# taha-kms/CLASSMATE-RAG

Hardware: AMD Instinct MI355X
Metric: hybrid queries/sec + recall@10 vs reference, 10M×768 chunks, 1/2/4/8 GPU (higher is better)
Workload: dtype fp32-accurate E5 (K10 f16x3 MFMA) + int8/f16/f64 dense + f64 BM25

## Files before the change

classmate-rag_amd/csrc/cm_bm25.hip:

```cpp
#include "cm_common.h"

#include <hipcub/hipcub.hpp>

#include <algorithm>
#include <cmath>
#include <cstdlib>
#include <numeric>
#include <vector>

namespace cm {

constexpr int kRange = 1024;
constexpr int kBmThreads = 256;
constexpr int kBoundsGroup = 8;
constexpr int kMergeThreads = 1024;
constexpr int kMergePer = 16;
constexpr int kTermLanesQd = 16;

__device__ inline int64_t lhead(int q, int64_t r, int64_t nr) { return (int64_t)q * nr + r; }
__host__ __device__ inline int64_t lheads_total(int nq, int64_t nr) { return (int64_t)nq * nr; }
__device__ inline int64_t lslot(int q, int64_t r, int64_t nr, int64_t nl, int k, int j) {
  return j == 0 ? lhead(q, r, nr) : nl + ((int64_t)q * nr + r) * (k - 1) + (j - 1);
}

// ... 937 lines not shown
  const int64_t d = df[i];
  double v = 0.0;
  if (t >= 0 && t < vocab && d > 0 && nc <= log_n) {
    v = logtab[nc - d] - logtab[d];
    if (v < 0) {
      const double e = eps_dev ? *eps_dev : __builtin_nan("");
      if (e != e) atomicOr(status, 1);
      v = e;
    }
  }
  q_idf[i] = v;
}

}

using namespace cm;

struct cm_bm25 {
  int dev = 0;
  hipStream_t stream = nullptr;
  int64_t ndocs = 0, npost = 0;
  int32_t vocab = 0;
  int64_t n_live = 0, sum_len = 0;
  double avgdl = 0.0, eps = 0.0;
  bool empty_vocab = false;
  DevBuf term_off, post_doc, post_tf, post_pos, dl, live, idf;
  DevBuf headtf, head_id;
  DevBuf logtab;
  int64_t log_n = -1;
  DevBuf head_maxtf, range_mindl;
  DevBuf blk_maxtf, blk_mindl;
  DevBuf blk_maxr;
  DevBuf blk16_maxr;
  double maxr_avgdl = 0.0;
  int32_t path = 0;
  int32_t last_rescored = 0;
  int32_t nhead = 0;
  int64_t npad = 0;
  int32_t lut_dmin = 0;
  double head_min_frac = 1.0 / 128.0;
  int64_t head_max_bytes = 8ll << 30;
  std::vector<double> idf_host;
  DevBuf ws, qbuf, obuf, allow_buf, tmp;
  KernelTimer timer;
  KernelTimer timer_b;
};

namespace {

inline double bm25_idf(int64_t n, int64_t df) {
  return std::log((double)(n - df) + 0.5) - std::log((double)df + 0.5);
}

int compute_idf_table(cm_bm25 *h, const std::vector<int32_t> &df, const std::vector<int32_t> &order) {
  h->idf_host.assign(h->vocab, 0.0);
  h->empty_vocab = false;
  h->eps = 0.0;
  h->avgdl = h->n_live ? (double)h->sum_len / (double)h->n_live : 0.0;
  if (h->n_live == 0) return CM_OK;
  if (order.empty()) {
    h->empty_vocab = true;
    return CM_OK;
  }
  double idf_sum = 0.0;
  for (int32_t t : order) {
    const double v = bm25_idf(h->n_live, df[t]);
// ... 52 lines not shown
    int32_t *dcand = h->tmp.as<int32_t>(), *dsat = dcand + cand.size();
    CM_HIP(hipMemcpyAsync(dcand, cand.data(), cand.size() * 4, hipMemcpyHostToDevice, h->stream));
    CM_HIP(hipMemsetAsync(dsat, 0, cand.size() * 4, h->stream));
    hipLaunchKernelGGL(bm25_head_sat_kernel, dim3(16, (unsigned)cand.size()), dim3(256), 0, h->stream, dcand,
                       (int)cand.size(), h->term_off.as<int64_t>(), h->post_tf.as<uint16_t>(), dsat);
    CM_HIP(hipGetLastError());
    std::vector<int32_t> sat(cand.size());
    CM_HIP(hipMemcpyAsync(sat.data(), dsat, cand.size() * 4, hipMemcpyDeviceToHost, h->stream));
    CM_HIP(hipStreamSynchronize(h->stream));
    size_t o = 0;
    for (size_t i = 0; i < cand.size(); ++i)
      if (!sat[i]) cand[o++] = cand[i];
    cand.resize(o);
  }
  const int64_t max_h = h->head_max_bytes / h->npad;
  if ((int64_t)cand.size() > max_h) cand.resize((size_t)std::max<int64_t>(max_h, 0));
  std::vector<int32_t> hid((size_t)std::max(h->vocab, 1), -1);
  for (size_t i = 0; i < cand.size(); ++i) hid[cand[i]] = (int32_t)i;
  if ((rc = h->head_id.ensure((size_t)std::max(h->vocab, 1) * 4))) return rc;
  CM_HIP(hipMemcpyAsync(h->head_id.ptr, hid.data(), (size_t)std::max(h->vocab, 1) * 4, hipMemcpyHostToDevice,
                        h->stream));
  if (!cand.empty()) {
    const size_t bytes = cand.size() * (size_t)h->npad;
    if ((rc = h->headtf.ensure(bytes)) || (rc = h->tmp.ensure(cand.size() * 4))) return rc;
    CM_HIP(hipMemsetAsync(h->headtf.ptr, 0, bytes, h->stream));
    CM_HIP(hipMemcpyAsync(h->tmp.ptr, cand.data(), cand.size() * 4, hipMemcpyHostToDevice, h->stream));
    hipLaunchKernelGGL(bm25_head_fill_kernel, dim3(64, (unsigned)cand.size()), dim3(256), 0, h->stream,
                       h->tmp.as<int32_t>(), (int)cand.size(), h->term_off.as<int64_t>(), h->post_doc.as<int32_t>(),
                       h->post_tf.as<uint16_t>(), h->headtf.as<uint8_t>(), h->npad);
    CM_HIP(hipGetLastError());
    CM_HIP(hipStreamSynchronize(h->stream));
  }
  h->nhead = (int32_t)cand.size();
  const int64_t nr = std::max<int64_t>(1, ceil_div(h->ndocs, kRange));
  if ((rc = h->range_mindl.ensure((size_t)nr * 4))) return rc;
  hipLaunchKernelGGL(bm25_range_mindl_kernel, dim3((unsigned)ceil_div(nr * 64, 256)), dim3(256), 0, h->stream,
                     h->dl.as<int32_t>(), h->ndocs, (int)nr, h->range_mindl.as<int32_t>());
  CM_HIP(hipGetLastError());
  const int64_t nblk = nr * (kRange / 64);
  if ((rc = h->blk_mindl.ensure((size_t)nblk * 4))) return rc;
  hipLaunchKernelGGL(bm25_blk_mindl_kernel, dim3((unsigned)ceil_div(nblk, 256)), dim3(256), 0, h->stream,
                     h->dl.as<int32_t>(), h->ndocs, nblk, h->blk_mindl.as<int32_t>());
  CM_HIP(hipGetLastError());
  if (h->nhead) {
    if ((rc = h->head_maxtf.ensure((size_t)h->nhead * nr)) || (rc = h->blk_maxtf.ensure((size_t)h->nhead * nblk)))
      return rc;
    hipLaunchKernelGGL(bm25_head_max_kernel, dim3((unsigned)ceil_div((int64_t)h->nhead * nr * 64, 256)), dim3(256), 0,
                       h->stream, h->headtf.as<uint8_t>(), h->npad, (int)nr, h->nhead, h->head_maxtf.as<uint8_t>());
    CM_HIP(hipGetLastError());
    hipLaunchKernelGGL(bm25_blk_max_kernel, dim3((unsigned)ceil_div((int64_t)h->nhead * nblk, 256)), dim3(256), 0,
                       h->stream, h->headtf.as<uint8_t>(), h->npad, nblk, h->nhead, h->blk_maxtf.as<uint8_t>());
    CM_HIP(hipGetLastError());
    h->maxr_avgdl = h->avgdl > 0.0 ? h->avgdl * 1.05 : 0.0;
    if (h->maxr_avgdl > 0.0) {
      if ((rc = h->blk_maxr.ensure((size_t)h->nhead * nblk)) || (rc = h->blk16_maxr.ensure((size_t)h->nhead * nblk * 4)))
        return rc;
      hipLaunchKernelGGL(bm25_blk_maxratio_kernel, dim3((unsigned)ceil_div((int64_t)h->nhead * nblk, 256)),
                         dim3(256), 0, h->stream, h->headtf.as<uint8_t>(), h->npad, h->dl.as<int32_t>(), h->ndocs,
                         nblk, h->nhead, h->maxr_avgdl, h->blk_maxr.as<uint8_t>(), 64);
      CM_HIP(hipGetLastError());
      hipLaunchKernelGGL(bm25_blk_maxratio_kernel, dim3((unsigned)ceil_div((int64_t)h->nhead * nblk * 4, 256)),
                         dim3(256), 0, h->stream, h->headtf.as<uint8_t>(), h->npad, h->dl.as<int32_t>(), h->ndocs,
                         nblk * 4, h->nhead, h->maxr_avgdl, h->blk16_maxr.as<uint8_t>(), 16);
      CM_HIP(hipGetLastError());
    }
  }
// ... 67 lines not shown
  off += 256;
  w.df = reinterpret_cast<int64_t *>(p + off);
  off += round_up((int64_t)std::max(total_terms, 1) * 8, 256);
  w.qd_code = reinterpret_cast<int32_t *>(p + off);
  off += round_up((int64_t)std::max(nq, 1) * kTermLanes * 4, 256);
  w.qd_idf = reinterpret_cast<double *>(p + off);
  off += round_up((int64_t)std::max(nq, 1) * kTermLanes * 8, 256);
  w.qd_tb = reinterpret_cast<int32_t *>(p + off);
  off += round_up((int64_t)std::max(nq, 1) * 4, 256);
  w.qd_len = reinterpret_cast<int32_t *>(p + off);
  off += round_up((int64_t)std::max(nq, 1) * 4, 256);
  w.qd_term = reinterpret_cast<int32_t *>(p + off);
  off += round_up((int64_t)std::max(nq, 1) * kTermLanes * 4, 256);
  w.total = off;
  return w;
}

#ifndef K2A_RPW
#define K2A_RPW 4
#endif
#ifndef K2B_GRID
#define K2B_GRID 2048
#endif
int bm25_launch_core(cm_bm25 *h, const int32_t *q_terms_dev, const int32_t *q_off_dev, int nq, int total_terms, int k,
                     const uint32_t *allow_dev, const BmWs &w, double *score_dev, int64_t *row_dev, hipStream_t st,
                     hipEvent_t gate = nullptr) {
  int rc;
  const double *avgdl = w.avgdl;
  const int nr = (int)std::max<int64_t>(1, ceil_div(h->ndocs, kRange));
  if (nr > kMergePer * kMergeThreads) CM_FAIL(CM_EUNSUPPORTED, "BM25 shard too large (> 16.7M docs)");
  const int ngroups = (nr + 1 + kBoundsGroup - 1) / kBoundsGroup;
  const int64_t nb = (int64_t)total_terms * ngroups;
  const bool prune = h->path != 1 && !(bm25_debug_flags() & 4);
  if (nq > 0) {
    hipLaunchKernelGGL(bm25_qcand_kernel, dim3((unsigned)ceil_div(nq, 256)), dim3(256), 0, st, q_terms_dev, q_off_dev,
                       nq, h->vocab, h->nhead ? h->head_id.as<int32_t>() : (const int32_t *)nullptr,
                       h->term_off.as<int64_t>(), (int)prune, w.qcand, w.q_idf, prune ? w.qd_code : nullptr,
                       w.qd_idf, w.qd_tb, w.qd_len, w.qd_term);
    CM_HIP(hipGetLastError());
  }
  if (nb > 0) {
    hipLaunchKernelGGL(bm25_bounds_kernel, dim3((unsigned)ceil_div(nb, 256)), dim3(256), 0, st, q_terms_dev,
                       total_terms, h->vocab, nr, h->term_off.as<int64_t>(), h->post_doc.as<int32_t>(), w.qcand,
                       w.bounds);
    CM_HIP(hipGetLastError());
  }
  CM_HIP(hipMemsetAsync(w.thr, 0xff, (size_t)nq * 8, st));
  if (prune && nq > 0 && env_knob("CM_BM25_TSEED", true)) {
    hipLaunchKernelGGL(bm25_tseed_kernel, dim3((unsigned)nq), dim3(kSeedThreads), 0, st, nq, k, w.qd_code,
                       w.qd_idf, w.qd_len, w.qd_term, h->term_off.as<int64_t>(), h->post_doc.as<int32_t>(),
                       h->post_tf.as<uint16_t>(), h->headtf.as<uint8_t>(), h->npad, h->dl.as<int32_t>(),
                       h->live.as<uint32_t>(), allow_dev, avgdl, w.thr);
    CM_HIP(hipGetLastError());
  }
  hipLaunchKernelGGL(bm25_lut_kernel, dim3(kLutW * kLutTF / 256), dim3(256), 0, st, (const double *)avgdl, h->lut_dmin,
                     w.lut);
  CM_HIP(hipGetLastError());
  const int64_t nqg = ceil_div(nq, kQPerWave);
  const int rpw = (int)std::min<int64_t>(kMaxRangesPerWave, std::max<int64_t>(1, nqg * nr / (256 * 4 * 24)));
  const int64_t nwaves = nqg * ceil_div(nr, rpw);
  const int64_t nblk = ceil_div(nwaves, kBmThreads / 64);
  const int rpw_a = std::max(1, std::min(rpw, (int)K2A_RPW));
  const int64_t nblk_a = ceil_div(nqg * ceil_div(nr, rpw_a), kBmThreads / 64);
  if (nblk > INT32_MAX || nblk_a > INT32_MAX) CM_FAIL(CM_EUNSUPPORTED, "BM25 batch too large");
  const int32_t *head_id = h->nhead ? h->head_id.as<int32_t>() : (const int32_t *)nullptr;
  if (gate) CM_HIP(hipStreamWaitEvent(st, gate, 0));
  h->timer.begin(st);
  if (prune) {
    hipLaunchKernelGGL(bm25_tail_kernel<uint16_t>, dim3((unsigned)nblk_a), dim3(kBmThreads), 0, st, q_terms_dev,
                       q_off_dev, nq, h->vocab, w.q_idf, w.bounds, nr, rpw_a, h->post_doc.as<int32_t>(),
                       h->post_tf.as<uint16_t>(), head_id, h->headtf.as<uint8_t>(), h->npad, h->dl.as<int32_t>(),
                       h->live.as<uint32_t>(), allow_dev, avgdl, k, w.cand_key, w.cand_row, w.thr, w.need, w.qd_code,
                       w.qd_term, w.qd_idf, w.qd_tb, w.qd_len,
                       (h->nhead && h->maxr_avgdl > 0.0) ? h->blk_maxr.as<uint8_t>() : (const uint8_t *)nullptr,
                       h->nhead ? h->blk_maxtf.as<uint8_t>() : (const uint8_t *)nullptr, h->blk_mindl.as<int32_t>(),
                       h->maxr_avgdl, (int64_t)nr * (kRange / 64),
                       h->nhead ? h->head_maxtf.as<uint8_t>() : (const uint8_t *)nullptr, h->range_mindl.as<int32_t>(),
                       bm25_debug_flags(),
                       (h->nhead && h->maxr_avgdl > 0.0) ? h->blk16_maxr.as<uint8_t>() : (const uint8_t *)nullptr);
    h->timer.end(st);
    CM_HIP(hipGetLastError());
    if ((rc = launch_bm25_merge(w.cand_key, w.cand_row, nq, nr, k, score_dev, row_dev, st))) return rc;
    CM_HIP(hipMemsetAsync(w.item_count, 0, 4, st));
    hipLaunchKernelGGL(bm25_plan_kernel, dim3((unsigned)ceil_div(nqg * nr, 256)), dim3(256), 0, st, w.qd_code,
                       w.qd_idf, w.qd_len, nq, (int)(head_id != nullptr), h->head_maxtf.as<uint8_t>(),
                       h->range_mindl.as<int32_t>(), h->blk_maxtf.as<uint8_t>(), h->blk_mindl.as<int32_t>(),
                       (h->nhead && h->maxr_avgdl > 0.0) ? h->blk_maxr.as<uint8_t>() : (const uint8_t *)nullptr,
                       h->maxr_avgdl, nr, (int64_t)nr * (kRange / 64), avgdl, k, score_dev, row_dev, w.need, w.items,
                       w.item_count,
                       (h->nhead && h->maxr_avgdl > 0.0 && !env_knob("CM_BM25_SUB16_OFF", false))
                           ? h->blk16_maxr.as<uint8_t>() : (const uint8_t *)nullptr,
                       w.items_sm);
    CM_HIP(hipGetLastError());
    h->timer_b.begin(st);
    hipLaunchKernelGGL(bm25_block_kernel, dim3(K2B_GRID), dim3(256), 0, st, w.items, w.item_count, w.qd_code,
                       w.qd_idf, w.qd_tb, w.bounds, nr, h->post_doc.as<int32_t>(), h->headtf.as<uint8_t>(), h->npad,
                       h->dl.as<int32_t>(), h->live.as<uint32_t>(), allow_dev, h->ndocs, avgdl, k, score_dev, nq,
                       w.cand_key, w.cand_row, w.items_sm);
    h->timer_b.end(st);
    CM_HIP(hipGetLastError());
  }
  hipLaunchKernelGGL(bm25_range_kernel<uint16_t>, dim3((unsigned)nblk), dim3(kBmThreads), 0, st, q_terms_dev,
                     q_off_dev, nq, w.q_idf, w.bounds, nr, rpw, h->term_off.as<int64_t>(), h->post_doc.as<int32_t>(),
                     h->post_tf.as<uint16_t>(), head_id, h->headtf.as<uint8_t>(), h->npad, h->dl.as<int32_t>(),
                     h->live.as<uint32_t>(), allow_dev, h->ndocs, avgdl, w.lut, h->lut_dmin, k, w.cand_key,
                     w.cand_row, w.thr, prune ? (const uint8_t *)w.need : (const uint8_t *)nullptr, h->vocab,
                     bm25_debug_flags());
  if (!prune) h->timer.end(st);
  CM_HIP(hipGetLastError());
  return launch_bm25_merge(w.cand_key, w.cand_row, nq, nr, k, score_dev, row_dev, st);
}

int32_t count_rescored(cm_bm25 *h, int nq, const BmWs &w, hipStream_t st) {
  const int64_t nr = std::max<int64_t>(1, ceil_div(h->ndocs, kRange));
  const int64_t n = ceil_div(std::max(nq, 1), kQPerWave) * nr;
  std::vector<uint8_t> v((size_t)n);
  uint32_t items = 0;
  if (hipMemcpyAsync(v.data(), w.need, (size_t)n, hipMemcpyDeviceToHost, st) != hipSuccess ||
      hipMemcpyAsync(&items, w.item_count, 4, hipMemcpyDeviceToHost, st) != hipSuccess ||
      hipStreamSynchronize(st) != hipSuccess)
    return -1;
  int64_t c = items;
  for (uint8_t b : v) c += __builtin_popcount(b);
  return (int32_t)std::min<int64_t>(c, INT32_MAX);
}

void bm25_free(cm_bm25 *h) {
  for (DevBuf *b : {&h->term_off, &h->post_doc, &h->post_tf, &h->post_pos, &h->dl, &h->live, &h->idf, &h->ws,
                    &h->qbuf, &h->obuf, &h->allow_buf, &h->tmp, &h->headtf, &h->head_id, &h->head_maxtf,
                    &h->range_mindl, &h->blk_maxtf, &h->blk_mindl, &h->blk_maxr, &h->blk16_maxr})
    b->release();
}

int bm25_search_full(cm_bm25 *h, const int32_t *q_terms, const int32_t *q_off, int nq, int k, const double *q_idf,
                     double avgdl, const uint32_t *allow_dev, int64_t n_cand, double *out_score, int64_t *out_row) {
  const int64_t n = std::max<int64_t>(h->ndocs, 1);
  int rc;
  size_t tmp_bytes = 0;
  CM_HIP(hipcub::DeviceRadixSort::SortPairs(nullptr, tmp_bytes, (const uint64_t *)nullptr, (uint64_t *)nullptr,
                                            (const int32_t *)nullptr, (int32_t *)nullptr, (int)n, 0, 64, h->stream));
  const size_t off1 = round_up((int64_t)tmp_bytes, 256);
  const size_t need = off1 + (size_t)round_up(n * 8, 256) * 3 + (size_t)round_up(n * 4, 256) * 2;
  if ((rc = h->ws.ensure(need))) return rc;
  char *base = h->ws.as<char>();
  double *score = reinterpret_cast<double *>(base + off1);
  uint64_t *keys = reinterpret_cast<uint64_t *>(base + off1 + round_up(n * 8, 256));
  uint64_t *skeys = reinterpret_cast<uint64_t *>(base + off1 + 2 * round_up(n * 8, 256));
  int32_t *rows = reinterpret_cast<int32_t *>(base + off1 + 3 * round_up(n * 8, 256));
  int32_t *srows = rows + round_up(n * 4, 256) / 4;
  const int64_t kk = std::min<int64_t>(k, n_cand);
  std::vector<uint64_t> hk((size_t)std::max<int64_t>(kk, 1));
  std::vector<int32_t> hr((size_t)std::max<int64_t>(kk, 1));
  for (int i = 0; i < nq; ++i) {
    CM_HIP(hipMemsetAsync(score, 0, (size_t)n * 8, h->stream));
    for (int32_t j = q_off[i]; j < q_off[i + 1]; ++j) {
      const int32_t t = q_terms[j];
      if (t < 0 || t >= h->vocab || q_idf[j] == 0.0) continue;
      int64_t lh[2];
      CM_HIP(hipMemcpyAsync(lh, h->term_off.as<int64_t>() + t, 16, hipMemcpyDeviceToHost, h->stream));
      CM_HIP(hipStreamSynchronize(h->stream));
      if (lh[1] <= lh[0]) continue;
      hipLaunchKernelGGL(bm25_scatter_term_kernel, dim3((unsigned)ceil_div(lh[1] - lh[0], 256)), dim3(256), 0,
                         h->stream, lh[0], lh[1], h->post_doc.as<int32_t>(), h->post_tf.as<uint16_t>(),
// ... 778 lines not shown
```

classmate-rag_amd/csrc/cm_bm25_prune.inc:

```

#ifndef K2A_CAP
#define K2A_CAP 320
#endif
#ifndef K2A_SUB
#define K2A_SUB 4
#endif
#ifndef K2B_U
#define K2B_U 2
#endif
#ifndef K2A_WPE
#define K2A_WPE 5
#endif
#ifndef K2A_PREB
#define K2A_PREB 0
#endif
#ifndef K2A_DLB
#define K2A_DLB 0
#endif
#ifndef K2A_BF
#define K2A_BF 0
#endif
#ifndef K2A_PACK
#define K2A_PACK 1
#endif
typedef uint16_t u16x2_t __attribute__((ext_vector_type(2)));
constexpr int kCandCap = K2A_CAP;

__device__ inline int lds_find(const int32_t *a, int n, int32_t x) {
  int lo = 0, hi = n;
  while (lo < hi) {
    const int mid = (lo + hi) >> 1;
    if (a[mid] < x) lo = mid + 1;
    else hi = mid;
  }
  return (lo < n && a[lo] == x) ? lo : -1;
}

constexpr float kPlanSlack = 1.0f + 2e-5f;
__device__ inline float idf_up(double x) { return x > 0.0 ? fmaxf(__double2float_ru(x), 1.2e-38f) : 0.0f; }
__device__ inline float inv_avg_lo(double avgdl) { return (float)(1.0 / avgdl) * (1.0f - 1e-6f); }
__device__ inline float kd_lo32(int32_t dlen, float inv_avg) { return 1.5f * (0.25f + 0.75f * (float)dlen * inv_avg); }
__device__ inline float ratio_up32(uint32_t tf, float kd) {
  const float t = (float)tf;
  return (t * 2.5f) * __builtin_amdgcn_rcpf(t + kd);
}
template <typename TF>
__global__ void __launch_bounds__(kBmThreads) __attribute__((amdgpu_waves_per_eu(K2A_WPE)))
    bm25_tail_kernel(const int32_t *__restrict__ q_terms, const int32_t *__restrict__ q_off, int nq, int32_t vocab,
                     const double *__restrict__ q_idf, const int64_t *__restrict__ bounds, int nr, int rpw,
                     const int32_t *__restrict__ post_doc, const TF *__restrict__ post_tf,
                     const int32_t *__restrict__ head_id, const uint8_t *__restrict__ headtf, int64_t npad,
                     const int32_t *__restrict__ dl, const uint32_t *__restrict__ live,
                     const uint32_t *__restrict__ allow, const double *__restrict__ avgdl_p, int k,
                     uint64_t *__restrict__ cand_key, uint32_t *__restrict__ cand_row,
                     unsigned long long *__restrict__ thr_key, uint8_t *__restrict__ need,
                     const int32_t *__restrict__ qd_code, const int32_t *__restrict__ qd_term,
                     const double *__restrict__ qd_idf, const int32_t *__restrict__ qd_tb,
                     const int32_t *__restrict__ qd_len, const uint8_t *__restrict__ blk_maxr,
                     const uint8_t *__restrict__ blk_maxtf, const int32_t *__restrict__ blk_mindl,
                     double maxr_avgdl, int64_t nblk, const uint8_t *__restrict__ head_maxtf,
                     const int32_t *__restrict__ range_mindl, int dbg, const uint8_t *__restrict__ blk16_maxr) {
  constexpr int W = kBmThreads / 64;
  const double avgdl = *avgdl_p;
  const bool use_r = blk_maxr != nullptr && avgdl <= maxr_avgdl;
  const uint8_t *blk_h = use_r ? blk_maxr : blk_maxtf;
  (void)blk_h;
#ifndef CM_ABLATION
  dbg = 0;
#endif
  __shared__ int32_t s_pdoc[W][kCandCap];
  __shared__ uint16_t s_ptf[W][kCandCap];
  __shared__ uint64_t s_key[W][kCandCap];
  __shared__ uint8_t s_eln[W][kCandCap];
  __shared__ int32_t s_t[W][64], s_h[W][64], s_off[W][64], s_cnt[W][64];
  __shared__ double s_idf[W][64];
  __shared__ float s_fi[W][64];
  __shared__ float s_hk[W][64];
  __shared__ double s_tq[W][kQPerWave];
#if K2A_PREB == 2
  __shared__ float s_hb[W][K2A_SUB][64];
  __shared__ float s_kdr[W][K2A_SUB];
#endif
  const float inv_avg = inv_avg_lo(avgdl);
  const int lane = threadIdx.x & 63;
  const int wave = threadIdx.x >> 6;
  const int nb = gridDim.x;
  const int b = blockIdx.x;
  const int per = nb >> 3, rem = nb & 7, x = b & 7, y = b >> 3;
  const int lb = (x < rem ? x * (per + 1) : rem * (per + 1) + (x - rem) * per) + y;
  const int nqg = (nq + kQPerWave - 1) / kQPerWave;
  const int wid = lb * W + wave;
  const int qg = wid % nqg;
  const int q0 = qg * kQPerWave;
  const int rg = wid / nqg;
  const int r0 = rg * rpw, r1 = min(r0 + rpw, nr);
  if (r0 >= r1) return;
  const int nqw = min(kQPerWave, nq - q0);
  int32_t *pdoc = s_pdoc[wave];
  uint16_t *ptf = s_ptf[wave];
  uint64_t *skey = s_key[wave];
  uint8_t *eln = s_eln[wave];
  int32_t *st = s_t[wave], *sh = s_h[wave], *soff = s_off[wave], *scnt = s_cnt[wave];
  double *sidf = s_idf[wave];
  const int64_t bstride = nr + 1;
  const int my_q = lane / kTermLanes, my_j = lane % kTermLanes;
  int my_tb = 0, my_L = 0, my_c = 0;
  int32_t my_t = -1;
  double my_idf = 0.0;
  if (my_q < nqw) {
    const int64_t di = (int64_t)(q0 + my_q) * kTermLanes + my_j;
    my_tb = qd_tb[q0 + my_q];
    my_L = qd_len[q0 + my_q];
    my_t = qd_term[di];
    my_c = qd_code[di];
    my_idf = qd_idf[di];
  }
  const bool q_ok = my_q < nqw && my_L <= kTermLanes;
  const uint64_t okb = __ballot(q_ok && my_j == 0);
  const uint32_t qokm = (uint32_t)((okb & 1u) | ((okb >> 15) & 2u) | ((okb >> 30) & 4u) | ((okb >> 45) & 8u));
  const bool has_term = q_ok && my_j < my_L;
  const int my_i = my_tb + my_j;
  if (!has_term) {
    my_t = -1;
    my_c = 0;
    my_idf = 0.0;
  }
  const int32_t my_h = (my_c & 0x3fffffff) - 1;
  const bool tail = my_t >= 0 && ((my_c >> 30) & 1);
  st[lane] = my_t;
  sh[lane] = my_h;
  sidf[lane] = my_idf;
  s_fi[wave][lane] = idf_up(my_idf);
  s_hk[wave][lane] = (use_r && my_h >= 0) ? (1.0f / 102.0f) : 0.0f;
  constexpr int SUB = K2A_SUB;
  constexpr int NG = kQPerWave * SUB;
  int64_t my_lo = 0, my_hi = 0;
  if (tail) {
    my_lo = bounds[(int64_t)my_i * bstride + r0];
    my_hi = bounds[(int64_t)my_i * bstride + min(r0 + SUB, r1)];
  }
  for (int r = r0; r < r1;) {
    int nsub = min(SUB, r1 - r);
    auto scan_counts = [&](int &cnt_, int &excl_, int &n_tot_) __attribute__((always_inline)) {
      cnt_ = (int)(my_hi - my_lo);
      int incl = cnt_;
#pragma unroll
      for (int o = 1; o < 64; o <<= 1) {
        const int v = __shfl_up(incl, o);
        if (lane >= o) incl += v;
      }
      excl_ = incl - cnt_;
      n_tot_ = __builtin_amdgcn_readlane(incl, 63);
    };
    int cnt, excl, n_tot;
    scan_counts(cnt, excl, n_tot);
    while (n_tot > kCandCap && nsub > 1) {
      nsub >>= 1;
      if (tail) my_hi = bounds[(int64_t)my_i * bstride + r + nsub];
      scan_counts(cnt, excl, n_tot);
    }
    int64_t nx_hi = my_hi;
    if (r + nsub < r1 && tail) nx_hi = bounds[(int64_t)my_i * bstride + min(r + nsub + SUB, r1)];
    uint64_t Tv = kEmptyKey;
    if (lane < nqw) Tv = __hip_atomic_load(thr_key + q0 + lane, __ATOMIC_RELAXED, __HIP_MEMORY_SCOPE_AGENT);
    if (lane < kQPerWave) s_tq[wave][lane] = Tv == kEmptyKey ? -INFINITY : f64_unorder(~Tv);
    if (n_tot > kCandCap) {
      if (lane < nsub) need[(int64_t)qg * nr + r + lane] = (uint8_t)qokm;
      if (lane < nqw * nsub) {
        const int qq = lane / nsub, sb = lane - qq * nsub;
        if ((qokm >> qq) & 1u) {
          const int64_t o = lhead(q0 + qq, r + sb, nr);
          cand_key[o] = kEmptyKey;
          cand_row[o] = 0xffffffffu;
        }
      }
      my_lo = my_hi;
      my_hi = nx_hi;
      r += nsub;
      continue;
    }
    if (lane < nsub) need[(int64_t)qg * nr + r + lane] = 0;
    soff[lane] = excl;
    scnt[lane] = cnt;
#if K2A_PREB == 2
    for (int sb = 0; sb < nsub; ++sb) {
      const float kdr = kd_lo32(range_mindl[r + sb], inv_avg);
      s_hb[wave][sb][lane] = my_h >= 0 ? s_fi[wave][lane] * ratio_up32(head_maxtf[(int64_t)my_h * nr + r + sb], kdr) : 0.0f;
      if (lane == 0) s_kdr[wave][sb] = kdr;
    }
#endif
    for (int e0 = 0; e0 < n_tot; e0 += 64) {
      const int e = e0 + lane;
      int lo = 0, hi = 63;
      while (lo < hi) {
        const int mid = (lo + hi + 1) >> 1;
        if (__shfl(excl, mid) <= e) lo = mid;
        else hi = mid - 1;
      }
// ... 115 lines not shown
            if (c > 0) {
              const int o = soff[l2];
              const int xx = lds_find(pdoc + o, c, d);
              if (xx >= 0) tf_set(jj, ptf[o + xx]);
            }
          }
        }
        const double Tq = s_tq[wave][qb / kTermLanes];
        float ub0 = 0.0f;
#pragma unroll
        for (int jj = 0; jj < kTermLanes; ++jj) {
          const uint32_t v = tf_get(jj);
          const float hk = s_hk[wave][qb + jj];
          const float rr = hk > 0.0f ? (float)v * hk : ratio_up32(v, kdb);
          if (v) ub0 += s_fi[wave][qb + jj] * rr;
        }
        bool pass = !((double)(ub0 * kPlanSlack) < Tq);
        int32_t dlen = 0;
        if (pass) {
#pragma unroll
          for (int jj = 0; jj < kTermLanes; ++jj) {
            const int32_t hh = sh[qb + jj];
            if (hh >= 0) tf_set(jj, (dbg & 64) ? 1u : (uint32_t)headtf[(int64_t)hh * npad + d]);
          }
          dlen = (dbg & 512) ? 120 : dl[d];
          float ub = 0.0f;
          const float kd32 = kd_lo32(dlen, inv_avg);
#pragma unroll
          for (int jj = 0; jj < kTermLanes; ++jj)
            if (tf_get(jj)) ub += s_fi[wave][qb + jj] * ratio_up32(tf_get(jj), kd32);
          pass = !((double)(ub * kPlanSlack) < Tq);
        }
#else
#if K2A_PACK
        u16x2_t tfp[kTermLanes / 2];
#pragma unroll
        for (int jj = 0; jj < kTermLanes; ++jj) {
          const int32_t hh = sh[qb + jj];
          tfp[jj >> 1][jj & 1] =
              hh >= 0 ? ((dbg & 64) ? (uint16_t)1 : (uint16_t)headtf[(int64_t)hh * npad + d]) : (uint16_t)0;
        }
        auto tf_get = [&](int jj) __attribute__((always_inline)) -> uint32_t { return tfp[jj >> 1][jj & 1]; };
        auto tf_set = [&](int jj, uint32_t v) __attribute__((always_inline)) { tfp[jj >> 1][jj & 1] = (uint16_t)v; };
#else
        uint32_t tfv[kTermLanes];
#pragma unroll
        for (int jj = 0; jj < kTermLanes; ++jj) {
          const int32_t hh = sh[qb + jj];
          tfv[jj] = hh >= 0 ? ((dbg & 64) ? 1u : (uint32_t)headtf[(int64_t)hh * npad + d]) : 0u;
        }
        auto tf_get = [&](int jj) __attribute__((always_inline)) -> uint32_t { return tfv[jj]; };
        auto tf_set = [&](int jj, uint32_t v) __attribute__((always_inline)) { tfv[jj] = v; };
#endif
#if K2A_DLB
        const int32_t bmin = blk_mindl[d >> 6];
#else
        const int32_t dlen = (dbg & 512) ? 120 : dl[d];
#endif
#pragma unroll
        for (int jj = 0; jj < kTermLanes; ++jj) {
          const int l2 = qb + jj;
          const int32_t t2 = st[l2];
          if (t2 < 0 || sh[l2] >= 0) continue;
          if (t2 == tj) {
            tf_set(jj, ptf[e]);
          } else {
            const int c = (dbg & 256) ? 0 : scnt[l2];
            if (c > 0) {
              const int o = soff[l2];
              const int xx = lds_find(pdoc + o, c, d);
              if (xx >= 0) tf_set(jj, ptf[o + xx]);
            }
          }
        }
        const double Tq = s_tq[wave][qb / kTermLanes];
#if K2A_DLB
        float ubb = 0.0f;
        const float kdb = kd_lo32(bmin, inv_avg);
#pragma unroll
        for (int jj = 0; jj < kTermLanes; ++jj)
          if (tf_get(jj)) ubb += s_fi[wave][qb + jj] * ratio_up32(tf_get(jj), kdb);
        bool pass = !((double)(ubb * kPlanSlack) < Tq);
        int32_t dlen = 0;
        if (pass) {
          dlen = (dbg & 512) ? 120 : dl[d];
          float ub = 0.0f;
          const float kd32 = kd_lo32(dlen, inv_avg);
#pragma unroll
          for (int jj = 0; jj < kTermLanes; ++jj)
            if (tf_get(jj)) ub += s_fi[wave][qb + jj] * ratio_up32(tf_get(jj), kd32);
          pass = !((double)(ub * kPlanSlack) < Tq);
        }
#else
        float ub = 0.0f;
        const float kd32 = kd_lo32(dlen, inv_avg);
#pragma unroll
        for (int jj = 0; jj < kTermLanes; ++jj)
          if (K2A_BF || tf_get(jj)) ub += s_fi[wave][qb + jj] * ratio_up32(tf_get(jj), kd32);
        const bool pass = !((double)(ub * kPlanSlack) < Tq);
#endif
#endif
        if (pass) {
          const double kd = kd_of(dlen, avgdl);
          double sc = 0.0;
#pragma unroll
          for (int jj = 0; jj < kTermLanes; ++jj) {
            const int l2 = qb + jj;
            if (st[l2] < 0) continue;
            if (tf_get(jj)) sc = sc + bm25_contrib_fast(sidf[l2], tf_get(jj), kd);
          }
          key = score_key(sc);
        }
      }
      skey[e] = key;
    }
    wave_lds_sync();
    int n_v = 0;
    for (int e0 = 0; e0 < ((dbg & 32) ? 0 : n_tot); e0 += 64) {
      const int e = e0 + lane;
      uint64_t key = kEmptyKey;
      uint32_t row = 0xffffffffu;
      int qe = 0, ge = 0;
      if (e < n_tot) {
        key = skey[e];
        row = (uint32_t)pdoc[e];
        qe = eln[e] >> 4;
        ge = qe * SUB + ((int)row / kRange - r);
      }
      const uint64_t Tq = (uint64_t)__shfl((long long)Tv, qe);
      const bool valid = key != kEmptyKey && key <= Tq;
      const uint64_t vm = __ballot(valid);
      const int pos = n_v + (int)__popcll(vm & ((1ull << lane) - 1ull));
      if (valid) {
        skey[pos] = key;
        pdoc[pos] = (int32_t)row;
        eln[pos] = (uint8_t)ge;
      }
      n_v += (int)__popcll(vm);
    }
    wave_lds_sync();
    int cq = 0;
    if (n_v <= 64) {
      const bool mine = lane < n_v;
      const uint64_t key = mine ? skey[lane] : kEmptyKey;
      const uint32_t row = mine ? (uint32_t)pdoc[lane] : 0xffffffffu;
      const int ge = mine ? eln[lane] : 255;
      int rank = 0;
      for (int xx = 0; xx < n_v; ++xx) {
        const int gx = eln[xx];
        rank += (gx == ge && pk_less(skey[xx], (uint32_t)pdoc[xx], key, row)) ? 1 : 0;
        cq += gx == lane ? 1 : 0;
      }
      cq = min(cq, k);
      if (mine && rank < k) {
        const int qe = ge / SUB;
        const int64_t o = lslot(q0 + qe, r + (ge - qe * SUB), nr, lheads_total(nq, nr), k, rank);
        cand_key[o] = key;
        cand_row[o] = row;
        if (rank == k - 1) atomicMin(thr_key + q0 + qe, (unsigned long long)key);
      }
    } else {
#pragma unroll 1
// ... 583 lines not shown

__global__ void bm25_head_max_kernel(const uint8_t *__restrict__ headtf, int64_t npad, int nr, int nhead,
                                     uint8_t *__restrict__ head_maxtf) {
  const int64_t w = ((int64_t)blockIdx.x * blockDim.x + threadIdx.x) >> 6;
  if (w >= (int64_t)nhead * nr) return;
  const int lane = threadIdx.x & 63;
  const int64_t hh = w / nr, r = w - hh * nr;
  const uint4 v = *reinterpret_cast<const uint4 *>(headtf + hh * npad + r * kRange + 16 * lane);
  const uint32_t wv[4] = {v.x, v.y, v.z, v.w};
  uint32_t m = 0;
#pragma unroll
  for (int u = 0; u < 4; ++u) {
    const uint32_t a = wv[u];
    m = max(m, max(max(a & 0xffu, (a >> 8) & 0xffu), max((a >> 16) & 0xffu, a >> 24)));
  }
  for (int o = 32; o > 0; o >>= 1) m = max(m, (uint32_t)__shfl_xor((int)m, o));
  if (lane == 0) head_maxtf[w] = (uint8_t)m;
}

__global__ void bm25_range_mindl_kernel(const int32_t *__restrict__ dl, int64_t ndocs, int nr,
                                        int32_t *__restrict__ range_mindl) {
  const int64_t w = ((int64_t)blockIdx.x * blockDim.x + threadIdx.x) >> 6;
  if (w >= nr) return;
  const int lane = threadIdx.x & 63;
  int32_t m = INT32_MAX;
  for (int u = 0; u < kRange / 64; ++u) {
    const int64_t d = w * kRange + u * 64 + lane;
    if (d < ndocs) m = min(m, dl[d]);
  }
  for (int o = 32; o > 0; o >>= 1) m = min(m, __shfl_xor(m, o));
  if (lane == 0) range_mindl[w] = m;
}

#ifndef K2S_CAP
#define K2S_CAP 1024
#endif
constexpr int kSeedCap = K2S_CAP;
constexpr int kSeedThreads = 256;
constexpr int kSeedPer = kSeedCap / kSeedThreads;
__global__ void __launch_bounds__(kSeedThreads) bm25_tseed_kernel(
    int nq, int k, const int32_t *__restrict__ qd_code, const double *__restrict__ qd_idf,
    const int32_t *__restrict__ qd_len, const int32_t *__restrict__ qd_term, const int64_t *__restrict__ term_off,
    const int32_t *__restrict__ post_doc, const uint16_t *__restrict__ post_tf, const uint8_t *__restrict__ headtf,
    int64_t npad, const int32_t *__restrict__ dl, const uint32_t *__restrict__ live,
    const uint32_t *__restrict__ allow, const double *__restrict__ avgdl_p,
    unsigned long long *__restrict__ thr_key) {
  const int q = blockIdx.x, tid = threadIdx.x, lane = tid & 63, wave = tid >> 6;
  if (q >= nq || k > kSeedCap) return;
  const int L = qd_len[q];
  if (L <= 0 || L > kTermLanes) return;
  __shared__ int32_t s_t[kTermLanes], s_h[kTermLanes];
  __shared__ double s_i[kTermLanes];
  __shared__ uint64_t sk[kSeedThreads / 64];
  __shared__ int s_gt, s_bad, s_n;
  __shared__ int64_t s_p0;
  if (wave == 0) {
    int32_t t = -1, code = 0;
    double idf = 0.0;
    if (lane < kTermLanes) {
      if (lane < L) {
        t = qd_term[(int64_t)q * kTermLanes + lane];
        code = qd_code[(int64_t)q * kTermLanes + lane];
        idf = qd_idf[(int64_t)q * kTermLanes + lane];
      }
      s_t[lane] = t;
      s_h[lane] = (code & 0x3fffffff) - 1;
      s_i[lane] = idf;
    }
    const bool bad = __ballot(lane < L && t >= 0 && idf < 0.0) != 0;
    const bool walked = lane < L && t >= 0 && ((code >> 30) & 1);
    int64_t df = walked ? term_off[t + 1] - term_off[t] : INT64_MAX;
    int best = walked ? lane : 64;
#pragma unroll
    for (int o = 32; o > 0; o >>= 1) {
      const int64_t odf = __shfl_xor(df, o);
      const int ob = __shfl_xor(best, o);
      if (odf < df || (odf == df && ob < best)) {
        df = odf;
        best = ob;
      }
    }
    const int32_t gt_all = __shfl(t, best < 64 ? best : 0);
    if (lane == 0) {
      s_bad = bad || best >= 64 || df < k;
      s_gt = best < 64 ? gt_all : -1;
      s_n = (int)min<int64_t>(df, kSeedCap);
      s_p0 = best < 64 ? term_off[gt_all] : 0;
    }
  }
  __syncthreads();
  if (s_bad) return;
  const int32_t gt = s_gt;
  const int n = s_n;
  const int64_t p0 = s_p0;
  const double avgdl = *avgdl_p;
  uint64_t kk[kSeedPer];
#pragma unroll
  for (int i = 0; i < kSeedPer; ++i) kk[i] = kEmptyKey;
#pragma unroll
  for (int u = 0; u < kSeedPer; ++u) {
    const int e = tid + u * kSeedThreads;
    if (e >= n) break;
    const int32_t d = post_doc[p0 + e];
    const uint32_t tfg = post_tf[p0 + e];
    const uint32_t aw = allow ? allow[d >> 5] : 0xffffffffu;
    const bool ok = ((live[d >> 5] & aw) >> (d & 31)) & 1u;
    const int32_t dlen = dl[d];
    uint32_t tf[kTermLanes];
#pragma unroll
    for (int j = 0; j < kTermLanes; ++j) {
      const int32_t h = s_h[j];
      tf[j] = (j < L && h >= 0) ? (uint32_t)headtf[(int64_t)h * npad + d] : 0u;
    }
    if (!ok) continue;
    const double kd = kd_of(dlen, avgdl);
    double sc = 0.0;
#pragma unroll
    for (int j = 0; j < kTermLanes; ++j) {
      if (j >= L) break;
      const int32_t tj = s_t[j];
      if (tj < 0) continue;
      const uint32_t v = tj == gt ? tfg : tf[j];
      if (v) sc = sc + bm25_contrib_fast(s_i[j], v, kd);
    }
    uint64_t ck = score_key(sc);
#pragma unroll
    for (int i = 0; i < kSeedPer; ++i) {
      if (ck < kk[i]) {
        const uint64_t tmp = kk[i];
        kk[i] = ck;
        ck = tmp;
      }
    }
  }
  uint64_t kth = kEmptyKey;
  for (int i = 0; i < k; ++i) {
    uint64_t m = kk[0];
#pragma unroll
    for (int o = 32; o > 0; o >>= 1) {
      const uint64_t om = __shfl_xor(m, o);
      m = om < m ? om : m;
    }
    if (lane == 0) sk[wave] = m;
    __syncthreads();
    m = sk[0];
// ... 22 lines not shown
```

Measured before the change: 34190.

## Add packed hot-head tf/doclen table and split short/long term slots in BM25

Adds an optional per-document 16/32-byte record packing doc length with the term frequencies of the first few head terms. The seed and prune kernels can then fetch them with one vector load instead of many strided headtf byte reads. The tail kernel also splits term slots into a short prefix and a long suffix that is only processed when some query in the wave has more terms. It also caches thresholds in shared memory instead of a shuffle. The hot table costs extra device memory and a build kernel, and it is gated behind an environment knob that defaults off.

```diff
diff --git a/classmate-rag_amd/csrc/cm_bm25.hip b/classmate-rag_amd/csrc/cm_bm25.hip
--- a/classmate-rag_amd/csrc/cm_bm25.hip
+++ b/classmate-rag_amd/csrc/cm_bm25.hip
@@ -993,6 +993,8 @@
   DevBuf blk_maxtf, blk_mindl;
   DevBuf blk_maxr;
   DevBuf blk16_maxr;
+  DevBuf hot;
+  bool hot_built = false;
   double maxr_avgdl = 0.0;
   int32_t path = 0;
   int32_t last_rescored = 0;
@@ -1111,6 +1113,15 @@
     CM_HIP(hipStreamSynchronize(h->stream));
   }
   h->nhead = (int32_t)cand.size();
+  h->hot_built = false;
+  if (env_knob("CM_BM25_HOT", false)) {
+    if ((rc = h->hot.ensure((size_t)h->npad * 16 * K2A_HOTQ))) return rc;
+    hipLaunchKernelGGL(bm25_hot_fill_kernel, dim3((unsigned)ceil_div(h->npad, 256)), dim3(256), 0, h->stream,
+                       h->dl.as<int32_t>(), h->headtf.as<uint8_t>(), h->npad, h->ndocs, (int)h->nhead,
+                       h->hot.as<uint4>());
+    CM_HIP(hipGetLastError());
+    h->hot_built = true;
+  }
   const int64_t nr = std::max<int64_t>(1, ceil_div(h->ndocs, kRange));
   if ((rc = h->range_mindl.ensure((size_t)nr * 4))) return rc;
   hipLaunchKernelGGL(bm25_range_mindl_kernel, dim3((unsigned)ceil_div(nr * 64, 256)), dim3(256), 0, h->stream,
@@ -1244,6 +1255,8 @@
   const int ngroups = (nr + 1 + kBoundsGroup - 1) / kBoundsGroup;
   const int64_t nb = (int64_t)total_terms * ngroups;
   const bool prune = h->path != 1 && !(bm25_debug_flags() & 4);
+  const uint4 *hot =
+      (h->hot_built && env_knob("CM_BM25_HOT", false)) ? h->hot.as<uint4>() : (const uint4 *)nullptr;
   if (nq > 0) {
     hipLaunchKernelGGL(bm25_qcand_kernel, dim3((unsigned)ceil_div(nq, 256)), dim3(256), 0, st, q_terms_dev, q_off_dev,
                        nq, h->vocab, h->nhead ? h->head_id.as<int32_t>() : (const int32_t *)nullptr,
@@ -1262,7 +1275,7 @@
     hipLaunchKernelGGL(bm25_tseed_kernel, dim3((unsigned)nq), dim3(kSeedThreads), 0, st, nq, k, w.qd_code,
                        w.qd_idf, w.qd_len, w.qd_term, h->term_off.as<int64_t>(), h->post_doc.as<int32_t>(),
                        h->post_tf.as<uint16_t>(), h->headtf.as<uint8_t>(), h->npad, h->dl.as<int32_t>(),
-                       h->live.as<uint32_t>(), allow_dev, avgdl, w.thr);
+                       h->live.as<uint32_t>(), allow_dev, avgdl, w.thr, hot);
     CM_HIP(hipGetLastError());
   }
   hipLaunchKernelGGL(bm25_lut_kernel, dim3(kLutW * kLutTF / 256), dim3(256), 0, st, (const double *)avgdl, h->lut_dmin,
@@ -1289,7 +1302,8 @@
                        h->maxr_avgdl, (int64_t)nr * (kRange / 64),
                        h->nhead ? h->head_maxtf.as<uint8_t>() : (const uint8_t *)nullptr, h->range_mindl.as<int32_t>(),
                        bm25_debug_flags(),
-                       (h->nhead && h->maxr_avgdl > 0.0) ? h->blk16_maxr.as<uint8_t>() : (const uint8_t *)nullptr);
+                       (h->nhead && h->maxr_avgdl > 0.0) ? h->blk16_maxr.as<uint8_t>() : (const uint8_t *)nullptr,
+                       hot);
     h->timer.end(st);
     CM_HIP(hipGetLastError());
     if ((rc = launch_bm25_merge(w.cand_key, w.cand_row, nq, nr, k, score_dev, row_dev, st))) return rc;
@@ -1340,7 +1354,7 @@
 void bm25_free(cm_bm25 *h) {
   for (DevBuf *b : {&h->term_off, &h->post_doc, &h->post_tf, &h->post_pos, &h->dl, &h->live, &h->idf, &h->ws,
                     &h->qbuf, &h->obuf, &h->allow_buf, &h->tmp, &h->headtf, &h->head_id, &h->head_maxtf,
-                    &h->range_mindl, &h->blk_maxtf, &h->blk_mindl, &h->blk_maxr, &h->blk16_maxr})
+                    &h->range_mindl, &h->blk_maxtf, &h->blk_mindl, &h->blk_maxr, &h->blk16_maxr, &h->hot})
     b->release();
 }
 
diff --git a/classmate-rag_amd/csrc/cm_bm25_prune.inc b/classmate-rag_amd/csrc/cm_bm25_prune.inc
--- a/classmate-rag_amd/csrc/cm_bm25_prune.inc
+++ b/classmate-rag_amd/csrc/cm_bm25_prune.inc
@@ -23,6 +23,22 @@
 #ifndef K2A_PACK
 #define K2A_PACK 1
 #endif
+#ifndef K2A_HOTQ
+#define K2A_HOTQ 1
+#endif
+static_assert(K2A_HOTQ == 1 || K2A_HOTQ == 2, "one or two 16-byte quarters");
+#ifndef K2A_SHORT
+#define K2A_SHORT 8
+#endif
+static_assert(K2A_SHORT % 2 == 0 && K2A_SHORT >= 2 && K2A_SHORT <= 14, "an even number of term slots, below 16");
+constexpr int kHotWords = 4 * K2A_HOTQ;
+constexpr int kHotHeads = 16 * K2A_HOTQ - 4;
+__device__ inline uint32_t hot_tf(const uint4 r0, const uint4 r1, int32_t hh) {
+  const int wd = (hh + 4) >> 2;
+  uint32_t v = wd == 1 ? r0.y : (wd == 2 ? r0.z : r0.w);
+  if (K2A_HOTQ > 1) v = wd == 4 ? r1.x : (wd == 5 ? r1.y : (wd == 6 ? r1.z : (wd == 7 ? r1.w : v)));
+  return (v >> ((hh & 3) * 8)) & 0xffu;
+}
 typedef uint16_t u16x2_t __attribute__((ext_vector_type(2)));
 constexpr int kCandCap = K2A_CAP;
 
@@ -59,9 +75,12 @@
                      const int32_t *__restrict__ qd_len, const uint8_t *__restrict__ blk_maxr,
                      const uint8_t *__restrict__ blk_maxtf, const int32_t *__restrict__ blk_mindl,
                      double maxr_avgdl, int64_t nblk, const uint8_t *__restrict__ head_maxtf,
-                     const int32_t *__restrict__ range_mindl, int dbg, const uint8_t *__restrict__ blk16_maxr) {
+                     const int32_t *__restrict__ range_mindl, int dbg, const uint8_t *__restrict__ blk16_maxr,
+                     const uint4 *__restrict__ hot) {
   constexpr int W = kBmThreads / 64;
   const double avgdl = *avgdl_p;
+  const int32_t hot_n = (K2A_PREB == 0 && K2A_DLB == 0 && hot != nullptr) ? kHotHeads : 0;
+  (void)hot_n;
   const bool use_r = blk_maxr != nullptr && avgdl <= maxr_avgdl;
   const uint8_t *blk_h = use_r ? blk_maxr : blk_maxtf;
   (void)blk_h;
@@ -77,13 +96,17 @@
   __shared__ float s_fi[W][64];
   __shared__ float s_hk[W][64];
   __shared__ double s_tq[W][kQPerWave];
+  __shared__ uint64_t s_tv[W][kQPerWave];
+#if K2A_HOTQ > 1
+  __shared__ uint8_t s_hq[W][kQPerWave];
+#endif
 #if K2A_PREB == 2
   __shared__ float s_hb[W][K2A_SUB][64];
   __shared__ float s_kdr[W][K2A_SUB];
 #endif
   const float inv_avg = inv_avg_lo(avgdl);
   const int lane = threadIdx.x & 63;
-  const int wave = threadIdx.x >> 6;
+  const int wave = __builtin_amdgcn_readfirstlane((int)(threadIdx.x >> 6));
   const int nb = gridDim.x;
   const int b = blockIdx.x;
   const int per = nb >> 3, rem = nb & 7, x = b & 7, y = b >> 3;
@@ -119,6 +142,8 @@
   const uint64_t okb = __ballot(q_ok && my_j == 0);
   const uint32_t qokm = (uint32_t)((okb & 1u) | ((okb >> 15) & 2u) | ((okb >> 30) & 4u) | ((okb >> 45) & 8u));
   const bool has_term = q_ok && my_j < my_L;
+  const bool wave_long = __ballot(has_term && my_j >= K2A_SHORT) != 0;
+  (void)wave_long;
   const int my_i = my_tb + my_j;
   if (!has_term) {
     my_t = -1;
@@ -132,6 +157,12 @@
   sidf[lane] = my_idf;
   s_fi[wave][lane] = idf_up(my_idf);
   s_hk[wave][lane] = (use_r && my_h >= 0) ? (1.0f / 102.0f) : 0.0f;
+#if K2A_HOTQ > 1
+  {
+    const uint64_t b2 = __ballot(my_h >= 12 && my_h < kHotHeads);
+    if (lane < kQPerWave) s_hq[wave][lane] = ((b2 >> (kTermLanes * lane)) & ((1ull << kTermLanes) - 1ull)) != 0;
+  }
+#endif
   constexpr int SUB = K2A_SUB;
   constexpr int NG = kQPerWave * SUB;
   int64_t my_lo = 0, my_hi = 0;
@@ -163,7 +194,10 @@
     if (r + nsub < r1 && tail) nx_hi = bounds[(int64_t)my_i * bstride + min(r + nsub + SUB, r1)];
     uint64_t Tv = kEmptyKey;
     if (lane < nqw) Tv = __hip_atomic_load(thr_key + q0 + lane, __ATOMIC_RELAXED, __HIP_MEMORY_SCOPE_AGENT);
-    if (lane < kQPerWave) s_tq[wave][lane] = Tv == kEmptyKey ? -INFINITY : f64_unorder(~Tv);
+    if (lane < kQPerWave) {
+      s_tq[wave][lane] = Tv == kEmptyKey ? -INFINITY : f64_unorder(~Tv);
+      s_tv[wave][lane] = Tv;
+    }
     if (n_tot > kCandCap) {
       if (lane < nsub) need[(int64_t)qg * nr + r + lane] = (uint8_t)qokm;
       if (lane < nqw * nsub) {
@@ -345,46 +379,85 @@
           pass = !((double)(ub * kPlanSlack) < Tq);
         }
 #else
-#if K2A_PACK
-        u16x2_t tfp[kTermLanes / 2];
-#pragma unroll
-        for (int jj = 0; jj < kTermLanes; ++jj) {
+        uint4 r0 = make_uint4(0u, 0u, 0u, 0u), r1 = r0;
+        if (hot_n) {
+          r0 = hot[(int64_t)d * K2A_HOTQ];
+#if K2A_HOTQ > 1
+          if (s_hq[wave][qb / kTermLanes]) r1 = hot[(int64_t)d * K2A_HOTQ + 1];
+#endif
+        }
+        auto cold_tf = [&](int jj) __attribute__((always_inline)) -> uint32_t {
           const int32_t hh = sh[qb + jj];
-          tfp[jj >> 1][jj & 1] =
-              hh >= 0 ? ((dbg & 64) ? (uint16_t)1 : (uint16_t)headtf[(int64_t)hh * npad + d]) : (uint16_t)0;
-        }
-        auto tf_get = [&](int jj) __attribute__((always_inline)) -> uint32_t { return tfp[jj >> 1][jj & 1]; };
-        auto tf_set = [&](int jj, uint32_t v) __attribute__((always_inline)) { tfp[jj >> 1][jj & 1] = (uint16_t)v; };
-#else
-        uint32_t tfv[kTermLanes];
-#pragma unroll
-        for (int jj = 0; jj < kTermLanes; ++jj) {
-          const int32_t hh = sh[qb + jj];
-          tfv[jj] = hh >= 0 ? ((dbg & 64) ? 1u : (uint32_t)headtf[(int64_t)hh * npad + d]) : 0u;
-        }
-        auto tf_get = [&](int jj) __attribute__((always_inline)) -> uint32_t { return tfv[jj]; };
-        auto tf_set = [&](int jj, uint32_t v) __attribute__((always_inline)) { tfv[jj] = v; };
-#endif
-#if K2A_DLB
-        const int32_t bmin = blk_mindl[d >> 6];
-#else
-        const int32_t dlen = (dbg & 512) ? 120 : dl[d];
-#endif
-#pragma unroll
-        for (int jj = 0; jj < kTermLanes; ++jj) {
+          return hh >= hot_n ? ((dbg & 64) ? 1u : (uint32_t)headtf[(int64_t)hh * npad + d]) : 0u;
+        };
+        auto tail_tf = [&](int jj, uint32_t &v) __attribute__((always_inline)) {
           const int l2 = qb + jj;
           const int32_t t2 = st[l2];
-          if (t2 < 0 || sh[l2] >= 0) continue;
+          if (t2 < 0 || sh[l2] >= 0) return;
           if (t2 == tj) {
-            tf_set(jj, ptf[e]);
+            v = ptf[e];
           } else {
             const int c = (dbg & 256) ? 0 : scnt[l2];
             if (c > 0) {
               const int o = soff[l2];
               const int xx = lds_find(pdoc + o, c, d);
-              if (xx >= 0) tf_set(jj, ptf[o + xx]);
+              if (xx >= 0) v = ptf[o + xx];
             }
           }
+        };
+        auto hot_slot = [&](int jj, uint32_t &v) __attribute__((always_inline)) {
+          const int32_t hh = sh[qb + jj];
+          const uint32_t b = (dbg & 64) ? 1u : hot_tf(r0, r1, hh);
+          v = (uint32_t)hh < (uint32_t)hot_n ? b : v;
+        };
+        uint32_t tlo[K2A_SHORT];
+#pragma unroll
+        for (int jj = 0; jj < K2A_SHORT; ++jj) tlo[jj] = cold_tf(jj);
+#if K2A_DLB
+        const int32_t bmin = blk_mindl[d >> 6];
+#else
+        const int32_t dlen = (dbg & 512) ? 120 : (hot_n ? (int32_t)r0.x : dl[d]);
+#endif
+#pragma unroll
+        for (int jj = 0; jj < K2A_SHORT; ++jj) tail_tf(jj, tlo[jj]);
+        if (hot_n) {
+#pragma unroll
+          for (int jj = 0; jj < K2A_SHORT; ++jj) hot_slot(jj, tlo[jj]);
+        }
+#if K2A_PACK
+        u16x2_t tfp[kTermLanes / 2];
+#pragma unroll
+        for (int jj = 0; jj < kTermLanes / 2; ++jj)
+          tfp[jj] = 2 * jj + 1 < K2A_SHORT ? u16x2_t{(uint16_t)tlo[2 * jj < K2A_SHORT ? 2 * jj : 0],
+                                                     (uint16_t)tlo[2 * jj + 1 < K2A_SHORT ? 2 * jj + 1 : 0]}
+                                           : u16x2_t{0, 0};
+#pragma unroll
+        for (int jj = 0; jj < K2A_SHORT / 2; ++jj) {
+          uint32_t pk = __builtin_bit_cast(uint32_t, tfp[jj]);
+          asm volatile("" : "+v"(pk));
+          tfp[jj] = __builtin_bit_cast(u16x2_t, pk);
+        }
+        auto tf_get = [&](int jj) __attribute__((always_inline)) -> uint32_t { return tfp[jj >> 1][jj & 1]; };
+        auto tf_set = [&](int jj, uint32_t v) __attribute__((always_inline)) { tfp[jj >> 1][jj & 1] = (uint16_t)v; };
+#else
+        uint32_t tfv[kTermLanes];
+#pragma unroll
+        for (int jj = 0; jj < kTermLanes; ++jj) tfv[jj] = jj < K2A_SHORT ? tlo[jj < K2A_SHORT ? jj : 0] : 0u;
+        auto tf_get = [&](int jj) __attribute__((always_inline)) -> uint32_t { return tfv[jj]; };
+        auto tf_set = [&](int jj, uint32_t v) __attribute__((always_inline)) { tfv[jj] = v; };
+#endif
+        if (wave_long) {
+          uint32_t thi[kTermLanes - K2A_SHORT];
+#pragma unroll
+          for (int jj = K2A_SHORT; jj < kTermLanes; ++jj) thi[jj - K2A_SHORT] = cold_tf(jj);
+#pragma unroll
+          for (int jj = K2A_SHORT; jj < kTermLanes; ++jj) tail_tf(jj, thi[jj - K2A_SHORT]);
+          if (hot_n) {
+#pragma unroll
+            for (int jj = K2A_SHORT; jj < kTermLanes; ++jj) hot_slot(jj, thi[jj - K2A_SHORT]);
+          }
+#pragma unroll
+          for (int jj = K2A_SHORT; jj < kTermLanes; ++jj) tf_set(jj, thi[jj - K2A_SHORT]);
         }
         const double Tq = s_tq[wave][qb / kTermLanes];
 #if K2A_DLB
@@ -440,7 +513,7 @@
         qe = eln[e] >> 4;
         ge = qe * SUB + ((int)row / kRange - r);
       }
-      const uint64_t Tq = (uint64_t)__shfl((long long)Tv, qe);
+      const uint64_t Tq = s_tv[wave][qe];
       const bool valid = key != kEmptyKey && key <= Tq;
       const uint64_t vm = __ballot(valid);
       const int pos = n_v + (int)__popcll(vm & ((1ull << lane) - 1ull));
@@ -1090,6 +1163,25 @@
   if (lane == 0) range_mindl[w] = m;
 }
 
+__global__ void __launch_bounds__(256)
+    bm25_hot_fill_kernel(const int32_t *__restrict__ dl, const uint8_t *__restrict__ headtf, int64_t npad,
+                         int64_t ndocs, int nhead, uint4 *__restrict__ hot) {
+  const int64_t d = (int64_t)blockIdx.x * blockDim.x + threadIdx.x;
+  if (d >= npad) return;
+  uint32_t w[kHotWords];
+#pragma unroll
+  for (int i = 0; i < kHotWords; ++i) w[i] = 0u;
+  if (d < ndocs) {
+    w[0] = (uint32_t)dl[d];
+#pragma unroll
+    for (int i = 0; i < kHotHeads; ++i)
+      if (i < nhead) w[(i + 4) >> 2] |= (uint32_t)headtf[(int64_t)i * npad + d] << (((i + 4) & 3) * 8);
+  }
+#pragma unroll
+  for (int qd = 0; qd < K2A_HOTQ; ++qd)
+    hot[d * K2A_HOTQ + qd] = make_uint4(w[4 * qd], w[4 * qd + 1], w[4 * qd + 2], w[4 * qd + 3]);
+}
+
 #ifndef K2S_CAP
 #define K2S_CAP 1024
 #endif
@@ -1102,8 +1194,9 @@
     const int32_t *__restrict__ post_doc, const uint16_t *__restrict__ post_tf, const uint8_t *__restrict__ headtf,
     int64_t npad, const int32_t *__restrict__ dl, const uint32_t *__restrict__ live,
     const uint32_t *__restrict__ allow, const double *__restrict__ avgdl_p,
-    unsigned long long *__restrict__ thr_key) {
+    unsigned long long *__restrict__ thr_key, const uint4 *__restrict__ hot) {
   const int q = blockIdx.x, tid = threadIdx.x, lane = tid & 63, wave = tid >> 6;
+  const int32_t hot_n = hot != nullptr ? kHotHeads : 0;
   if (q >= nq || k > kSeedCap) return;
   const int L = qd_len[q];
   if (L <= 0 || L > kTermLanes) return;
@@ -1112,6 +1205,9 @@
   __shared__ uint64_t sk[kSeedThreads / 64];
   __shared__ int s_gt, s_bad, s_n;
   __shared__ int64_t s_p0;
+#if K2A_HOTQ > 1
+  __shared__ int s_q2;
+#endif
   if (wave == 0) {
     int32_t t = -1, code = 0;
     double idf = 0.0;
@@ -1125,6 +1221,13 @@
       s_h[lane] = (code & 0x3fffffff) - 1;
       s_i[lane] = idf;
     }
+#if K2A_HOTQ > 1
+    {
+      const int32_t hq = (code & 0x3fffffff) - 1;
+      const bool any2 = __ballot(lane < L && hq >= 12 && hq < kHotHeads) != 0;
+      if (lane == 0) s_q2 = any2;
+    }
+#endif
     const bool bad = __ballot(lane < L && t >= 0 && idf < 0.0) != 0;
     const bool walked = lane < L && t >= 0 && ((code >> 30) & 1);
     int64_t df = walked ? term_off[t + 1] - term_off[t] : INT64_MAX;
@@ -1163,12 +1266,26 @@
     const uint32_t tfg = post_tf[p0 + e];
     const uint32_t aw = allow ? allow[d >> 5] : 0xffffffffu;
     const bool ok = ((live[d >> 5] & aw) >> (d & 31)) & 1u;
-    const int32_t dlen = dl[d];
+    uint4 r0 = make_uint4(0u, 0u, 0u, 0u), r1 = r0;
+    if (hot_n) {
+      r0 = hot[(int64_t)d * K2A_HOTQ];
+#if K2A_HOTQ > 1
+      if (s_q2) r1 = hot[(int64_t)d * K2A_HOTQ + 1];
+#endif
+    }
+    const int32_t dlen = hot_n ? (int32_t)r0.x : dl[d];
     uint32_t tf[kTermLanes];
 #pragma unroll
     for (int j = 0; j < kTermLanes; ++j) {
       const int32_t h = s_h[j];
-      tf[j] = (j < L && h >= 0) ? (uint32_t)headtf[(int64_t)h * npad + d] : 0u;
+      tf[j] = (j < L && h >= hot_n) ? (uint32_t)headtf[(int64_t)h * npad + d] : 0u;
+    }
+    if (hot_n) {
+#pragma unroll
+      for (int j = 0; j < kTermLanes; ++j) {
+        const int32_t h = s_h[j];
+        if (j < L && (uint32_t)h < (uint32_t)hot_n) tf[j] = hot_tf(r0, r1, h);
+      }
     }
     if (!ok) continue;
     const double kd = kd_of(dlen, avgdl);
```

New measurement: 34200 (median of 2 runs). No clear change (+0.0%).
